# kohjingyu/gill

Measured on AMD Instinct MI355X. Metric: 512x512 images/sec/node, OPT-6.7B+SD1.5 50-step, higher is better.
Workload: dtype bf16

## Files before the change

### gill_amd/csrc/gemm.hip

```cpp
#include "ops.h"
#include <stdlib.h>

#define BM_HOST 128
#define BK 64
#define GEMM_THREADS 256
#define LN_MAX_PLANES 20

#define ZERO_PAGE_STEPS 127
__device__ __attribute__((aligned(256))) uint32_t g_zero_page_storage[(ZERO_PAGE_STEPS + 1) * 32];

const bf16_t* gill_zero_page() {
  static const bf16_t* p = nullptr;
  if (!p) {
    void* d = nullptr;
    if (hipGetSymbolAddress(&d, HIP_SYMBOL(g_zero_page_storage)) == hipSuccess) {
      (void)hipMemset(d, 0, sizeof(g_zero_page_storage));
      p = (const bf16_t*)d;
    }
  }
  return p;
}

struct GemmDev {
  GemmArgs a;
// ... 237 lines not shown

struct GemmTileCtx {
  int bx, by, bz, gdx, gdy;
  unsigned* seam_in = nullptr; unsigned seam_in_target = 0; int seam_in_mtg = 1; int prefetch = 0;
  unsigned* seam_out = nullptr;
};
template <int NWV, int BN, int CONV, int EPI, int STAGES, int KT, int MI, int SEAM = 0>
__device__ __forceinline__ void gemm_tile(const GemmDev& d, const GemmTileCtx cx) {
  constexpr int BM = (NWV / 2) * MI * 16;
  static_assert(MI == 4 || (MI == 2 && NWV == 4 && CONV == 0 && (STAGES == 2 || STAGES == 3) && KT == 64) ||
                    (MI == 2 && NWV == 8 && BN == 160 && STAGES == 3 && KT == 64) || (MI == 2 && NWV == 8 && BN == 64 && STAGES == 6 && CONV == 0 && KT == 64) ||
                    (MI == 2 && NWV == 8 && BN == 128 && STAGES == 2 && CONV == 0 && KT == 64),
                "MI = 2: the 4-wave 64-row plain tile, the 128 x 160 ping-pong tile (8 waves of 32 x 80), or the 128 x 64 streaming tile on 8 waves of 32 x 32");
  constexpr int NT = BN / 32;
  constexpr bool PP = (NWV == 8 && BN == 160 && STAGES == 3 && KT == 64);
  constexpr bool WBLK = (BN == 64 && STAGES == 6 && CONV == 0);
  static_assert(KT == 64 || KT == 32, "stage depth");
  constexpr int LPR = KT / 8;
  constexpr int RPI = 64 / LPR;
  constexpr int KK = KT / 32;
#define SWZ(row) (KT == 64 ? ((row) & 7) : (((row) >> 2) & 3))
  extern __shared__ __attribute__((aligned(16))) unsigned char smem_raw[];
  bf16_t* smem = reinterpret_cast<bf16_t*>(smem_raw);
  constexpr int A_ELEMS = BM * KT;
  constexpr int B_ELEMS = BN * KT;
  constexpr int BUF_ELEMS = A_ELEMS + B_ELEMS;

  const GemmArgs& p = d.a;
  const int tid = threadIdx.x;
  const int lane = tid & 63;
  const int w = __builtin_amdgcn_readfirstlane(tid >> 6);
  int tile;
  {
    const int nwg = cx.gdx, bid = cx.bx;
    const int q = nwg >> 3, r = nwg & 7;
    const int xcd = bid & 7, idx = bid >> 3;
    tile = (xcd < r ? xcd * (q + 1) : r * (q + 1) + (xcd - r) * q) + idx;
  }
  int gn = d.n_major ? tile / d.tiles_m : tile % d.groups_n;
  int tm = d.n_major ? tile % d.tiles_m : tile / d.groups_n;
  if (d.xb_m > 0) {
    const int bid = cx.bx, xcd = bid & 7, idx = bid >> 3;
    const int blocks_m = d.tiles_m / d.xb_m;
    const int bmi = xcd % blocks_m, bni = xcd / blocks_m;
    tm = bmi * d.xb_m + idx % d.xb_m;
    gn = bni * d.xb_n + idx / d.xb_m;
  }
  const int m0 = tm * BM;
  const int tn_first = gn * d.npw;
  const int ntl = (CONV != 0 || EPI == 2 || EPI == 7) ? 1 : ((d.tiles_n - tn_first < d.npw) ? d.tiles_n - tn_first : d.npw);
  int n0 = tn_first * BN;
  const int z = cx.by;
  const int kt_beg = z * d.ksteps_per_split;
  int kt_end = kt_beg + d.ksteps_per_split;
  if (kt_end > d.ksteps) kt_end = d.ksteps;
  const int nsteps = kt_end - kt_beg;
  const int cls = (CONV == 3) ? cx.bz : 0;
  const int ups_py = cls >> 1, ups_px = cls & 1;

  const int srow = lane / LPR;
  const int schunk = (lane % LPR) ^ SWZ(srow);

  constexpr int AI = BM / (RPI * NWV);
  int a_off1[AI], a_off2[AI], a_fl[AI], a_pc[AI];
#pragma unroll
  for (int i = 0; i < AI; ++i) {
    int row = (i * NWV + w) * RPI + srow;
    int m = m0 + row;
    if (m > p.M - 1) m = p.M - 1;
    a_fl[i] = 0; a_pc[i] = 0;
    if constexpr (CONV == 0) {
      a_off1[i] = m * p.lda + schunk * 8;
      a_off2[i] = m * p.lda2 + schunk * 8;
    } else {
      const int ohw = p.OH * p.OW;
      const int b = m / ohw;
      const int r = m - b * ohw;
      const int oy = r / p.OW;
      const int ox = r - oy * p.OW;
      int fl = 0, pc;
      if constexpr (CONV == 3) {
        const int shw = p.IH * p.IW;
        const int sb = m / shw;
        const int sr = m - sb * shw;
        const int sy = sr / p.IW, sx = sr - sy * p.IW;
        pc = m;
        fl |= (sy - 1 >= 0) ? 1 : 0; fl |= (sy + 1 < p.IH) ? 2 : 0;
        fl |= (sx - 1 >= 0) ? 4 : 0; fl |= (sx + 1 < p.IW) ? 8 : 0;
      } else if constexpr (CONV == 2) {
        pc = (b * p.IH + (oy >> 1)) * p.IW + (ox >> 1);
        fl |= (oy - 1 >= 0) ? 1 : 0; fl |= (oy + 1 < p.OH) ? 2 : 0;
        fl |= (ox - 1 >= 0) ? 4 : 0; fl |= (ox + 1 < p.OW) ? 8 : 0;
        fl |= (oy & 1) << 4; fl |= (ox & 1) << 5;
      } else {
        const int cy = oy * p.stride, cx = ox * p.stride;
        pc = (b * p.IH + cy) * p.IW + cx;
        fl |= (cy - 1 >= 0) ? 1 : 0; fl |= (cy + 1 < p.IH) ? 2 : 0;
        fl |= (cx - 1 >= 0) ? 4 : 0; fl |= (cx + 1 < p.IW) ? 8 : 0;
      }
      a_fl[i] = fl;
      a_pc[i] = m;
      a_off1[i] = pc * p.K1 + schunk * 8;
      a_off2[i] = pc * (p.Cin - p.K1) + schunk * 8;
    }
  }
  constexpr int WG = BN / RPI;
  constexpr int WI = (WG + NWV - 1) / NWV;
  static_assert(BN % RPI == 0, "whole row groups");
  const bool w_last_ok = ((WI - 1) * NWV + w) < WG;
  const int lw = AI + (w_last_ok ? WI : WI - 1);
  const bf16_t* w_ptr[WI];
  int n_issue = n0;
  auto tile_col = [&](int R) -> int {
    const int half = R / (BN / 2), q = R - half * (BN / 2);
    const int j = q >> 4, x = q & 15;
    int c;
    if constexpr (EPI == 1) {
      static_assert(EPI != 1 || NT % 4 == 0, "GEGLU: whole value/gate quads per wave");
      const int o = (x >> 2) * 8 + ((j >> 1) & 1) * 4 + (x & 3);
      c = (j >> 2) * 64 + (o >> 4) * 32 + (o & 15) + (j & 1) * 16;
    } else {
      c = ((j | 1) < NT) ? (j >> 1) * 32 + (x >> 2) * 8 + (j & 1) * 4 + (x & 3) : q;
    }
    return half * (BN / 2) + c;
  };
  const bool wblk = WBLK || (CONV == 0 && p.w_blk64 != 0);
  const int w_step = wblk ? 4096 : KT;
  const bf16_t* Wb = p.W + (p.wb_rows ? (size_t)(m0 / p.wb_rows) * (size_t)p.wb_stride : (size_t)0);
  auto w_setup = [&]() {
#pragma unroll
    for (int i = 0; i < WI; ++i) {
      int row = tile_col((i * NWV + w) * RPI + srow);
      int n = n_issue + row;
      if (n > p.N - 1) n = p.N - 1;
      if (wblk) w_ptr[i] = Wb + ((size_t)(n >> 6) * d.ksteps + kt_beg) * 4096 + (n & 63) * 64 + schunk * 8;
      else w_ptr[i] = Wb + ((size_t)cls * p.N + n) * p.K + schunk * 8 + kt_beg * KT;
    }
  };
  w_setup();
  const bf16_t* zero_lane = d.zero + schunk * 8;

  const bf16_t* a_ptr[AI];
  int seg_left = 0;
  auto seg_setup = [&](int k0) {
    if constexpr (CONV == 0) {
      const bool first = (k0 < p.K1);
      const bf16_t* src = first ? p.A : p.A2;
      const int kk = first ? k0 : k0 - p.K1;
#pragma unroll
      for (int i = 0; i < AI; ++i) a_ptr[i] = src + (first ? a_off1[i] : a_off2[i]) + kk;
      seg_left = ((first ? p.K1 : p.K) - k0) / KT;
    } else {
      if (CONV == 1 && k0 >= 9 * p.Cin) {
        const int ke = k0 - 9 * p.Cin;
        const bool fx = (ke < p.KX1);
        const bf16_t* xs = fx ? p.X1 : p.X2;
        const int cx = fx ? p.KX1 : (p.KX - p.KX1);
        const int kc = (fx ? ke : ke - p.KX1) + schunk * 8;
#pragma unroll
        for (int i = 0; i < AI; ++i) a_ptr[i] = xs + (size_t)a_pc[i] * cx + kc;
        seg_left = ((fx ? p.KX1 : p.KX) - ke) / KT;
      } else {
        int tap, c0;
        if (p.k_chunked) {
          const int chunk = k0 / (9 * BK);
          const int r = k0 - chunk * (9 * BK);
          tap = r / BK;
          c0 = chunk * BK + (r - tap * BK);
        } else {
          tap = k0 / p.Cin;
          c0 = k0 - tap * p.Cin;
        }
        const int ty = tap / 3;
        int dy = ty - 1, dx = tap - ty * 3 - 1;
        if constexpr (CONV == 3) { dy = ups_py - 1 + (tap >> 1); dx = ups_px - 1 + (tap & 1); }
        const int need = (dy < 0 ? 1 : (dy > 0 ? 2 : 0)) | (dx < 0 ? 4 : (dx > 0 ? 8 : 0));
        const bool first = (c0 < p.K1);
        const bf16_t* src = first ? p.A : p.A2;
        const int cs = first ? p.K1 : (p.Cin - p.K1);
        const int cc = first ? c0 : c0 - p.K1;
        const int delta = (dy * p.IW + dx) * cs + cc;
#pragma unroll
        for (int i = 0; i < AI; ++i) {
          int off = (first ? a_off1[i] : a_off2[i]);
          if constexpr (CONV == 2) {
            const int ddy = (dy + ((a_fl[i] >> 4) & 1)) >> 1, ddx = (dx + ((a_fl[i] >> 5) & 1)) >> 1;
            off += (ddy * p.IW + ddx) * cs + cc;
          } else {
            off += delta;
          }
          const bool ok = (a_fl[i] & need) == need;
          a_ptr[i] = ok ? src + off : zero_lane;
        }
        seg_left = p.k_chunked ? 1 : ((first ? p.K1 : p.Cin) - c0) / KT;
      }
    }
  };
  int k_issue = kt_beg * KT;
  int steps_in_tile = 0;
  auto issue_prepare = [&]() {
    if (steps_in_tile == nsteps) {
      steps_in_tile = 0;
      k_issue = kt_beg * KT;
      seg_left = 0;
      n_issue += BN;
      w_setup();
    }
    if (seg_left == 0) seg_setup(k_issue);
  };
  auto issue_dma = [&](int buf) {
    bf16_t* As = smem + buf * BUF_ELEMS;
    bf16_t* Bs = As + A_ELEMS;
#pragma unroll
    for (int i = 0; i < AI; ++i) {
      bf16_t* l = As + (i * NWV + w) * RPI * KT;
      __builtin_amdgcn_global_load_lds((const __attribute__((address_space(1))) void*)a_ptr[i],
                                       (__attribute__((address_space(3))) void*)l, 16, 0, 0);
    }
#pragma unroll
    for (int i = 0; i < WI; ++i) {
      if (i == WI - 1 && !w_last_ok) break;
      bf16_t* l = Bs + (i * NWV + w) * RPI * KT;
      __builtin_amdgcn_global_load_lds((const __attribute__((address_space(1))) void*)w_ptr[i],
                                       (__attribute__((address_space(3))) void*)l, 16, 0, WBLK ? 2 : 0);
    }
  };
  auto issue_dma_a = [&](int buf) {
    bf16_t* As = smem + buf * BUF_ELEMS;
#pragma unroll
    for (int i = 0; i < AI; ++i)
      __builtin_amdgcn_global_load_lds((const __attribute__((address_space(1))) void*)a_ptr[i],
                                       (__attribute__((address_space(3))) void*)(As + (i * NWV + w) * RPI * KT), 16, 0, 0);
  };
  auto issue_dma_w = [&](int buf, int koff) {
    bf16_t* Bs = smem + buf * BUF_ELEMS + A_ELEMS;
#pragma unroll
    for (int i = 0; i < WI; ++i) {
      if (i == WI - 1 && !w_last_ok) break;
      __builtin_amdgcn_global_load_lds((const __attribute__((address_space(1))) void*)(w_ptr[i] + koff),
                                       (__attribute__((address_space(3))) void*)(Bs + (i * NWV + w) * RPI * KT), 16, 0, 0);
    }
  };
  auto issue_post = [&]() {
    ++steps_in_tile;
    --seg_left;
#pragma unroll
    for (int i = 0; i < AI; ++i) a_ptr[i] += KT;
#pragma unroll
    for (int i = 0; i < WI; ++i) w_ptr[i] += WBLK ? 4096 : (CONV == 0 ? w_step : KT);
    k_issue += KT;
  };
  auto issue = [&](int buf) {
    issue_prepare();
    issue_dma(buf);
    issue_post();
  };

  f32x4 acc[MI][NT];

  const int wm = w >> 1, wn = w & 1;
  const int frow = lane & 15;
  const int fkc = lane >> 4;

  static_assert(STAGES >= 2 && STAGES <= 6, "ring depth");
  const int total_steps = ntl * nsteps;
  if constexpr (SEAM != 0) {
    static_assert(SEAM == 0 || (PP && !WBLK), "SEAM: the ping-pong tiles");
    if (cx.seam_in) {
      if (cx.prefetch) {
#pragma unroll
        for (int s = 0; s < STAGES - 1; ++s)
          if (s < total_steps) issue_dma_w(s, s * KT);
      }
      if (tid == 0) {
        unsigned* c = cx.seam_in + tm / cx.seam_in_mtg;
        for (unsigned spins = 0; __hip_atomic_load(c, __ATOMIC_RELAXED, __HIP_MEMORY_SCOPE_AGENT) < cx.seam_in_target && spins < COOP_SPIN_LIMIT; ++spins)
          __builtin_amdgcn_s_sleep(2);
        __builtin_amdgcn_fence(__ATOMIC_ACQUIRE, "agent");
      }
      __builtin_amdgcn_s_barrier();
#pragma unroll
      for (int s = 0; s < STAGES - 1; ++s)
        if (s < total_steps) { issue_prepare(); issue_dma_a(s); if (!cx.prefetch) issue_dma_w(s, 0); issue_post(); }
    } else {
#pragma unroll
      for (int s = 0; s < STAGES - 1; ++s)
        if (s < total_steps) issue(s);
    }
  } else {
#pragma unroll
  for (int s = 0; s < STAGES - 1; ++s)
    if (s < total_steps) issue(s);
  }
  float ln_rr[4] = {1.f, 1.f, 1.f, 1.f}, ln_rm[4] = {0.f, 0.f, 0.f, 0.f};
  if constexpr (EPI == 1 || EPI == 3 || EPI == 5) {
    if (p.ln_stats) {
#pragma unroll
      for (int i = 0; i < MI; ++i) {
        const int m = m0 + wm * (MI * 16) + i * 16 + frow;
        if (m < p.M) ln_row_factors(p, m, ln_rr[i], ln_rm[i]);
      }
    }
  }
  int buf = 0, buf_issue = STAGES - 1;
  int flat = 0;
  constexpr bool DEFER = (CONV == 0 && STAGES == 2 && !PP && (EPI == 1 || EPI == 3));
  int deferred_buf = -1;
  for (int t = 0; t < ntl; ++t, n0 += BN) {
#pragma unroll
  for (int i = 0; i < MI; ++i)
#pragma unroll
    for (int j = 0; j < NT; ++j) acc[i][j] = (f32x4){0.f, 0.f, 0.f, 0.f};
  if constexpr (PP) {
    const int grp = w >> 2;
    int issued = total_steps < STAGES - 1 ? total_steps : STAGES - 1;
    bf16x8 af[KK][MI];
    bf16x8 bfr[KK][NT];
    auto landed = [&](int k) {
      if (k >= nsteps) return;
      if constexpr (SEAM != 0) {
        if (cx.seam_in && cx.prefetch && k == 0 && issued == STAGES - 1) { asm volatile("s_waitcnt vmcnt(%0)" ::"n"(AI) : "memory"); return; }
      }
      if (issued - 1 - k <= 0) asm volatile("s_waitcnt vmcnt(0)" ::: "memory");
      else if (w_last_ok) asm volatile("s_waitcnt vmcnt(%0)" ::"n"(AI + WI) : "memory");
      else asm volatile("s_waitcnt vmcnt(%0)" ::"n"(AI + WI - 1) : "memory");
    };
    auto mem = [&](int k) {
      const int sb = k % STAGES;
      const bf16_t* As = smem + sb * BUF_ELEMS;
      const bf16_t* Bs = As + A_ELEMS;
#pragma unroll
      for (int kk = 0; kk < KK; ++kk) {
#pragma unroll
        for (int i = 0; i < MI; ++i) {
          const int row = wm * (MI * 16) + i * 16 + frow;
          af[kk][i] = *reinterpret_cast<const bf16x8*>(As + row * KT + (((kk * 4 + fkc) ^ SWZ(row)) * 8));
        }
#pragma unroll
        for (int j = 0; j < NT; ++j) {
          const int row = wn * (BN / 2) + j * 16 + frow;
          bfr[kk][j] = *reinterpret_cast<const bf16x8*>(Bs + row * KT + (((kk * 4 + fkc) ^ SWZ(row)) * 8));
        }
      }
      if (k + STAGES - 1 < nsteps) { issue_dma((k + STAGES - 1) % STAGES); ++issued; }
    };
    auto mma = [&](int k) {
      issue_post();
#pragma unroll
      for (int kk = 0; kk < KK; ++kk)
#pragma unroll
        for (int i = 0; i < MI; ++i)
#pragma unroll
          for (int j = 0; j < NT; ++j)
            acc[i][j] = __builtin_amdgcn_mfma_f32_16x16x32_bf16(bfr[kk][j], af[kk][i], acc[i][j], 0, 0, 0);
#pragma unroll
      for (int q = 0; q < KK * MI * NT; ++q) {
        __builtin_amdgcn_sched_group_barrier(0x008, 1, 0);
        __builtin_amdgcn_sched_group_barrier(0x006, 1, 0);
      }
      if (k + STAGES < nsteps) issue_prepare();
    };
    if (STAGES - 1 < nsteps) issue_prepare();
    landed(0);
    __builtin_amdgcn_s_barrier();
    if (grp == 0) {
      for (int k = 0; k < nsteps; ++k) {
        mem(k);
        __builtin_amdgcn_sched_barrier(0);
        __builtin_amdgcn_s_barrier();
        mma(k);
        landed(k + 1);
        __builtin_amdgcn_sched_barrier(0);
        __builtin_amdgcn_s_barrier();
      }
      __builtin_amdgcn_s_barrier();
    } else {
      __builtin_amdgcn_s_barrier();
      for (int k = 0; k < nsteps; ++k) {
        mem(k);
        landed(k + 1);
        __builtin_amdgcn_sched_barrier(0);
        __builtin_amdgcn_s_barrier();
        mma(k);
        __builtin_amdgcn_sched_barrier(0);
        __builtin_amdgcn_s_barrier();
      }
    }
  } else
  for (int it = 0; it < nsteps; ++it, ++flat) {
    if constexpr (STAGES == 2) {
      asm volatile("s_waitcnt vmcnt(0)" ::: "memory");
    } else if constexpr (STAGES == 3) {
      if (total_steps - 1 - flat <= 0) asm volatile("s_waitcnt vmcnt(0)" ::: "memory");
      else if (w_last_ok) asm volatile("s_waitcnt vmcnt(%0)" ::"n"(AI + WI) : "memory");
      else asm volatile("s_waitcnt vmcnt(%0)" ::"n"(AI + WI - 1) : "memory");
    } else {
      if (total_steps - 1 - flat < STAGES - 2) asm volatile("s_waitcnt vmcnt(0)" ::: "memory");
      else if (w_last_ok) asm volatile("s_waitcnt vmcnt(%0)" ::"n"((STAGES - 2) * (AI + WI)) : "memory");
      else asm volatile("s_waitcnt vmcnt(%0)" ::"n"((STAGES - 2) * (AI + WI - 1)) : "memory");
    }
    __builtin_amdgcn_s_barrier();
    const bf16_t* As = smem + buf * BUF_ELEMS;
    const bf16_t* Bs = As + A_ELEMS;
    buf = (buf + 1 == STAGES) ? 0 : buf + 1;
    bf16x8 af[KK][MI];
    bf16x8 bfr[KK][NT];
    auto frag_load = [&](int kk) {
#pragma unroll
      for (int i = 0; i < MI; ++i) {
        const int row = wm * (MI * 16) + i * 16 + frow;
        const int slot = (kk * 4 + fkc) ^ SWZ(row);
        af[kk][i] = *reinterpret_cast<const bf16x8*>(As + row * KT + slot * 8);
      }
#pragma unroll
      for (int j = 0; j < NT; ++j) {
        const int row = wn * (BN / 2) + j * 16 + frow;
        const int slot = (kk * 4 + fkc) ^ SWZ(row);
        bfr[kk][j] = *reinterpret_cast<const bf16x8*>(Bs + row * KT + slot * 8);
      }
    };
    frag_load(0);
    if (flat + STAGES - 1 < total_steps) {
      if (DEFER && it == nsteps - 1) deferred_buf = buf_issue;
      else issue(buf_issue);
    }
    buf_issue = (buf_issue + 1 == STAGES) ? 0 : buf_issue + 1;
#pragma unroll
    for (int kk = 0; kk < KK; ++kk) {
      if (kk + 1 < KK) {
        __builtin_amdgcn_sched_barrier(0);
        frag_load(kk + 1);
        __builtin_amdgcn_sched_barrier(0);
      }
#pragma unroll
      for (int i = 0; i < MI; ++i)
#pragma unroll
        for (int j = 0; j < NT; ++j)
          acc[i][j] = __builtin_amdgcn_mfma_f32_16x16x32_bf16(bfr[kk][j], af[kk][i], acc[i][j], 0, 0, 0);
    }
  }

  const int mrow = m0 + wm * (MI * 16) + frow;
  const int nbase = n0 + wn * (BN / 2);
  constexpr int NG = (NT + 1) / 2;
  auto out_row = [&](int m) -> int {
    if constexpr (CONV == 3) {
      const int shw = p.IH * p.IW;
      const int sb = m / shw;
      const int sr = m - sb * shw;
      const int sy = sr / p.IW, sx = sr - sy * p.IW;
      return (sb * p.OH + 2 * sy + ups_py) * p.OW + 2 * sx + ups_px;
    } else {
      return m;
    }
  };
  if constexpr (EPI == 2 || EPI == 7) {
    float* ws = p.ws + (size_t)z * (CONV == 3 ? 4 : 1) * p.M * p.N;
#pragma unroll
    for (int i = 0; i < MI; ++i) {
      if (mrow + i * 16 >= p.M) continue;
      const int m = out_row(mrow + i * 16);
#pragma unroll
      for (int g = 0; g < NG; ++g) {
        const bool pair = (2 * g + 1 < NT);
        const int j1 = pair ? 2 * g + 1 : 2 * g;
        const int n = nbase + (pair ? g * 32 + fkc * 8 : (2 * g) * 16 + fkc * 4);
        if (n >= p.N) continue;
        float* dst = ws + (size_t)m * p.N + n;
        if constexpr (EPI == 7) {
          st_wt_f32x4(dst, acc[i][2 * g]);
          if (pair && n + 4 < p.N) st_wt_f32x4(dst + 4, acc[i][j1]);
        } else {
          *reinterpret_cast<float4*>(dst) = make_float4(acc[i][2 * g][0], acc[i][2 * g][1], acc[i][2 * g][2], acc[i][2 * g][3]);
          if (pair && n + 4 < p.N)
            *reinterpret_cast<float4*>(dst + 4) = make_float4(acc[i][j1][0], acc[i][j1][1], acc[i][j1][2], acc[i][j1][3]);
        }
      }
    }
    if constexpr (EPI == 7) {
      static_assert(EPI != 7 || (PP && BN % 40 == 0), "COOP split-K finish: the ping-pong tiles");
      asm volatile("s_waitcnt vmcnt(0)" ::: "memory");
      __syncthreads();
      const int rpb = p.rows_per_batch;
      const int mtg = rpb > BM ? rpb / BM : 1, spg = rpb < BM ? BM / rpb : 1;
      const int G = mtg * cx.gdy;
      const int tg = tm / mtg;
      unsigned char* cs = smem_raw + 16384;
      float2 (*part)[10] = reinterpret_cast<float2 (*)[10]>(cs);
      float2* quad = reinterpret_cast<float2*>(cs + 2048);
      float2* mr = reinterpret_cast<float2*>(cs + 2304);
      unsigned* okf = reinterpret_cast<unsigned*>(cs + 2560);
      if (tid == 0) {
        const bool ok = coop_arrive_wait(p.coop_ctr + (size_t)tg * d.tiles_n + n0 / BN, (unsigned)G);
        __builtin_amdgcn_fence(__ATOMIC_ACQUIRE, "agent");
        *okf = ok ? 1u : 0u;
      }
      __syncthreads();
      const bool poison = *okf == 0u;
      constexpr int UPT = BN / 40;
      const int widx = z * mtg + (tm - tg * mtg);
      for (int u = widx; u < spg * UPT; u += G) {
        const int b = tg * spg + u / UPT, col0 = n0 + (u % UPT) * 40;
        if (rpb == 256) splitk_finish_unit<16, 40>(p, b, col0, tid, part, quad, mr, poison);
        else splitk_finish_unit<4, 40>(p, b, col0, tid, part, quad, mr, poison);
        __syncthreads();
      }
      if constexpr (SEAM != 0) {
        if (cx.seam_out) {
          asm volatile("s_waitcnt vmcnt(0)" ::: "memory");
          __syncthreads();
          if (tid == 0) {
            __builtin_amdgcn_fence(__ATOMIC_RELEASE, "agent");
            asm volatile("s_waitcnt vmcnt(0)" ::: "memory");
            __hip_atomic_fetch_add(cx.seam_out + tg, 1u, __ATOMIC_RELAXED, __HIP_MEMORY_SCOPE_AGENT);
          }
        }
      }
    }
  } else if constexpr (EPI == 1) {
    const float* rr = ln_rr; const float* rm = ln_rm;
#pragma unroll
    for (int qd = 0; qd < NT / 4; ++qd) {
      const int ol = fkc * 8;
      const int pv = nbase + qd * 64 + (ol >> 4) * 32 + (ol & 15);
      if (nbase + qd * 64 >= p.N) continue;
      const int no = (nbase + qd * 64) / 2 + ol;
      float4 bv[2], bg[2], sv[2], sg[2];
#pragma unroll
      for (int h = 0; h < 2; ++h) {
        bv[h] = p.bias ? *reinterpret_cast<const float4*>(p.bias + pv + 4 * h) : make_float4(0, 0, 0, 0);
        bg[h] = p.bias ? *reinterpret_cast<const float4*>(p.bias + pv + 16 + 4 * h) : make_float4(0, 0, 0, 0);
        sv[h] = p.ln_stats ? *reinterpret_cast<const float4*>(p.ln_colsum + pv + 4 * h) : make_float4(0, 0, 0, 0);
        sg[h] = p.ln_stats ? *reinterpret_cast<const float4*>(p.ln_colsum + pv + 16 + 4 * h) : make_float4(0, 0, 0, 0);
      }
      __builtin_amdgcn_s_waitcnt(0x0F70);
      if (DEFER && qd == NT / 4 - 1 && deferred_buf >= 0) { issue(deferred_buf); deferred_buf = -1; }
#pragma unroll
      for (int i = 0; i < MI; ++i) {
        const int m = mrow + i * 16;
        float o[8];
#pragma unroll
        for (int h = 0; h < 2; ++h) {
          const f32x4 av = acc[i][qd * 4 + 2 * h], ag = acc[i][qd * 4 + 2 * h + 1];
          o[4 * h + 0] = (av[0] * rr[i] - rm[i] * sv[h].x + bv[h].x) * gelu_erf(ag[0] * rr[i] - rm[i] * sg[h].x + bg[h].x);
          o[4 * h + 1] = (av[1] * rr[i] - rm[i] * sv[h].y + bv[h].y) * gelu_erf(ag[1] * rr[i] - rm[i] * sg[h].y + bg[h].y);
          o[4 * h + 2] = (av[2] * rr[i] - rm[i] * sv[h].z + bv[h].z) * gelu_erf(ag[2] * rr[i] - rm[i] * sg[h].z + bg[h].z);
          o[4 * h + 3] = (av[3] * rr[i] - rm[i] * sv[h].w + bv[h].w) * gelu_erf(ag[3] * rr[i] - rm[i] * sg[h].w + bg[h].w);
        }
        uint4 ov; ov.x = pack_bf2(o[0], o[1]); ov.y = pack_bf2(o[2], o[3]); ov.z = pack_bf2(o[4], o[5]); ov.w = pack_bf2(o[6], o[7]);
        if (m < p.M) *reinterpret_cast<uint4*>((bf16_t*)p.C + (size_t)m * p.ldc + no) = ov;
      }
    }
  } else if constexpr (EPI == 5) {
    static_assert(EPI != 5 || BN == 160, "softmax epilogue: one 80-column head per wave half");
    const size_t vb = p.wb_rows ? (size_t)(m0 / p.wb_rows) * (size_t)p.vb_stride : (size_t)0;
    const float* bias = p.bias + vb;
    const float* csum = p.ln_colsum + vb;
    float4 bzs[NG][2], css[NG][2];
#pragma unroll
    for (int g = 0; g < NG; ++g) {
      const bool pair = (2 * g + 1 < NT);
      const int n = nbase + (pair ? g * 32 + fkc * 8 : (2 * g) * 16 + fkc * 4);
      bzs[g][0] = *reinterpret_cast<const float4*>(bias + n);
      css[g][0] = *reinterpret_cast<const float4*>(csum + n);
      bzs[g][1] = pair ? *reinterpret_cast<const float4*>(bias + n + 4) : make_float4(0, 0, 0, 0);
      css[g][1] = pair ? *reinterpret_cast<const float4*>(csum + n + 4) : make_float4(0, 0, 0, 0);
    }
    __builtin_amdgcn_s_waitcnt(0x0F70);
#pragma unroll
    for (int i = 0; i < MI; ++i) {
      const int m = mrow + i * 16;
      const float rr = ln_rr[i], rm = ln_rm[i];
      float v[NG][8];
      float mx = -INFINITY;
#pragma unroll
      for (int g = 0; g < NG; ++g) {
        const bool pair = (2 * g + 1 < NT);
        const f32x4 a0 = acc[i][2 * g], a1 = acc[i][pair ? 2 * g + 1 : 2 * g];
        v[g][0] = a0[0] * rr - rm * css[g][0].x + bzs[g][0].x; v[g][1] = a0[1] * rr - rm * css[g][0].y + bzs[g][0].y;
        v[g][2] = a0[2] * rr - rm * css[g][0].z + bzs[g][0].z; v[g][3] = a0[3] * rr - rm * css[g][0].w + bzs[g][0].w;
        v[g][4] = pair ? a1[0] * rr - rm * css[g][1].x + bzs[g][1].x : -INFINITY; v[g][5] = pair ? a1[1] * rr - rm * css[g][1].y + bzs[g][1].y : -INFINITY;
        v[g][6] = pair ? a1[2] * rr - rm * css[g][1].z + bzs[g][1].z : -INFINITY; v[g][7] = pair ? a1[3] * rr - rm * css[g][1].w + bzs[g][1].w : -INFINITY;
#pragma unroll
        for (int e = 0; e < 8; ++e) mx = fmaxf(mx, v[g][e]);
      }
      mx = fmaxf(mx, __shfl_xor(mx, 16, 64));
      mx = fmaxf(mx, __shfl_xor(mx, 32, 64));
      float sum = 0.f;
#pragma unroll
      for (int g = 0; g < NG; ++g)
#pragma unroll
        for (int e = 0; e < 8; ++e) { v[g][e] = __builtin_amdgcn_exp2f(v[g][e] - mx); sum += v[g][e]; }
      sum += __shfl_xor(sum, 16, 64);
      sum += __shfl_xor(sum, 32, 64);
      const float inv = 1.f / sum;
      if (m < p.M) {
        bf16_t* crow = (bf16_t*)p.C + (size_t)m * p.ldc;
#pragma unroll
        for (int g = 0; g < NG; ++g) {
          const bool pair = (2 * g + 1 < NT);
          const int n = nbase + (pair ? g * 32 + fkc * 8 : (2 * g) * 16 + fkc * 4);
          uint4 o; o.x = pack_bf2(v[g][0] * inv, v[g][1] * inv); o.y = pack_bf2(v[g][2] * inv, v[g][3] * inv);
          o.z = pack_bf2(v[g][4] * inv, v[g][5] * inv); o.w = pack_bf2(v[g][6] * inv, v[g][7] * inv);
          if (pair) *reinterpret_cast<uint4*>(crow + n) = o;
          else *reinterpret_cast<uint2*>(crow + n) = make_uint2(o.x, o.y);
        }
      }
    }
  } else if constexpr (EPI == 3) {
    int rq[MI], rk[MI], rv[MI]; bool mok[MI];
    float rr[MI], rm[MI];
#pragma unroll
    for (int i = 0; i < MI; ++i) {
      const int m = mrow + i * 16;
      mok[i] = m < p.M;
      rr[i] = p.ln_stats ? ln_rr[i] : p.alpha; rm[i] = ln_rm[i];
      const int b = m / p.ntok, t = m - b * p.ntok;
      rq[i] = (b * p.heads * p.ntok_pad_q + t) * p.dp;
      rk[i] = (b * p.heads * p.ntok_pad_kv + t + p.kv_tok_offset) * p.dp;
      rv[i] = b * p.heads * p.dpv * p.ntok_pad_kv + t + p.kv_tok_offset;
    }
    const int hd = p.heads * p.dp;
    float4 bzs[NG][2], css[NG][2];
#pragma unroll
    for (int g = 0; g < NG; ++g) {
      const bool pair = (2 * g + 1 < NT);
      const int n = nbase + (pair ? g * 32 + fkc * 8 : (2 * g) * 16 + fkc * 4);
      const bool hi = pair && (n + 4 < p.N);
#pragma unroll
      for (int e = 0; e < 2; ++e) {
        const bool ok = (n < p.N) && ((e == 0) || hi);
        bzs[g][e] = (p.bias && ok) ? *reinterpret_cast<const float4*>(p.bias + n + 4 * e) : make_float4(0, 0, 0, 0);
        css[g][e] = (p.ln_stats && ok) ? *reinterpret_cast<const float4*>(p.ln_colsum + n + 4 * e) : make_float4(0, 0, 0, 0);
      }
    }
    __builtin_amdgcn_s_waitcnt(0x0F70);
    if (DEFER && deferred_buf >= 0) { issue(deferred_buf); deferred_buf = -1; }
#pragma unroll
    for (int g = 0; g < NG; ++g) {
      const bool pair = (2 * g + 1 < NT);
      const int j1 = pair ? 2 * g + 1 : 2 * g;
      const int n = nbase + (pair ? g * 32 + fkc * 8 : (2 * g) * 16 + fkc * 4);
      if (n >= p.N) continue;
      const bool hi = pair && (n + 4 < p.N);
      const int segl = n / hd;
      const int within = n - segl * hd;
      const int h = within / p.dp, dd = within - h * p.dp;
      const int seg = p.seg_base + segl;
      const float4* bz = bzs[g]; const float4* cs = css[g];
#pragma unroll
      for (int i = 0; i < MI; ++i) {
        if (!mok[i]) continue;
        float v[8];
        const f32x4 a0 = acc[i][2 * g], a1 = acc[i][j1];
        v[0] = a0[0] * rr[i] - rm[i] * cs[0].x + bz[0].x; v[1] = a0[1] * rr[i] - rm[i] * cs[0].y + bz[0].y;
        v[2] = a0[2] * rr[i] - rm[i] * cs[0].z + bz[0].z; v[3] = a0[3] * rr[i] - rm[i] * cs[0].w + bz[0].w;
        v[4] = a1[0] * rr[i] - rm[i] * cs[1].x + bz[1].x; v[5] = a1[1] * rr[i] - rm[i] * cs[1].y + bz[1].y;
        v[6] = a1[2] * rr[i] - rm[i] * cs[1].z + bz[1].z; v[7] = a1[3] * rr[i] - rm[i] * cs[1].w + bz[1].w;
        if (seg == 0) {
#pragma unroll
          for (int e = 0; e < 8; ++e) v[e] *= p.qscale;
        }
        if (seg <= 1) {
          bf16_t* dst = (seg == 0) ? p.Cq + (size_t)rq[i] + (size_t)h * p.ntok_pad_q * p.dp + dd
                                   : p.Ck + (size_t)rk[i] + (size_t)h * p.ntok_pad_kv * p.dp + dd;
          if (hi) {
            uint4 o; o.x = pack_bf2(v[0], v[1]); o.y = pack_bf2(v[2], v[3]); o.z = pack_bf2(v[4], v[5]); o.w = pack_bf2(v[6], v[7]);
            *reinterpret_cast<uint4*>(dst) = o;
          } else {
            uint2 o; o.x = pack_bf2(v[0], v[1]); o.y = pack_bf2(v[2], v[3]);
            *reinterpret_cast<uint2*>(dst) = o;
          }
        } else {
          bf16_t* base = p.Cvt + (size_t)rv[i] + (size_t)(h * p.dpv + dd) * p.ntok_pad_kv;
          const int ne = hi ? 8 : 4;
#pragma unroll
          for (int e = 0; e < 8; ++e)
            if (e < ne) base[(size_t)e * p.ntok_pad_kv] = f2bf(v[e]);
          if (dd + ne == p.dp && p.dpv > p.dp) base[(size_t)ne * p.ntok_pad_kv] = (bf16_t)0x3F80;
        }
      }
    }
  } else {
    int crow[MI], rrow[MI]; bool mok[MI];
#pragma unroll
    for (int i = 0; i < MI; ++i) {
      const int m = mrow + i * 16;
      mok[i] = m < p.M;
      const int mc = mok[i] ? m : p.M - 1;
      crow[i] = out_row(mc) * p.ldc;
      rrow[i] = mc * p.ldr;
    }
    float2* red = reinterpret_cast<float2*>(smem);
    float2* red_lane = red + wm * BN + wn * (BN / 2);
    if (p.gn_stats) __syncthreads();
    float rws[4] = {0.f, 0.f, 0.f, 0.f}, rwq[4] = {0.f, 0.f, 0.f, 0.f};
    constexpr bool F32_PATHS = (CONV == 0 && EPI != 4);
    constexpr bool ALL_UPFRONT = !F32_PATHS;
    constexpr int NSLOT = ALL_UPFRONT ? NG : 1;
    const int wrow0 = m0 + wm * (MI * 16);
    const int wrow1 = (wrow0 + MI * 16 - 1 < p.M) ? wrow0 + MI * 16 - 1 : p.M - 1;
    const bool rv_pre = p.rowvec && wrow0 < p.M && (wrow0 / p.rows_per_batch == wrow1 / p.rows_per_batch);
    const bool rv_slow = p.rowvec && !rv_pre;
    const bool rf_slow = F32_PATHS && p.resid && p.resid_f32;
    const bool rb_pre = p.resid && !rf_slow;
    const float* colvec = rv_pre ? p.rowvec + (wrow0 / p.rows_per_batch) * p.rowvec_bstride : p.bias;
    const float* colvec2 = rv_pre ? p.bias : nullptr;
    float4 cv[NSLOT][2];
    uint2 rb[NSLOT][MI][2];
    auto load_group = [&](int g, int sl) {
      const bool pair = (2 * g + 1 < NT);
      const int n = nbase + (pair ? g * 32 + fkc * 8 : (2 * g) * 16 + fkc * 4);
      const bool hi = pair && (n + 4 < p.N);
      const int nl = (n < p.N) ? n : 0;
      const int nh = hi ? n + 4 : nl;
      cv[sl][0] = cv[sl][1] = make_float4(0, 0, 0, 0);
      if (colvec) {
        cv[sl][0] = *reinterpret_cast<const float4*>(colvec + nl);
        cv[sl][1] = *reinterpret_cast<const float4*>(colvec + nh);
      }
      if (colvec2) {
        const float4 t0 = *reinterpret_cast<const float4*>(colvec2 + nl);
        const float4 t1 = *reinterpret_cast<const float4*>(colvec2 + nh);
        cv[sl][0].x += t0.x; cv[sl][0].y += t0.y; cv[sl][0].z += t0.z; cv[sl][0].w += t0.w;
        cv[sl][1].x += t1.x; cv[sl][1].y += t1.y; cv[sl][1].z += t1.z; cv[sl][1].w += t1.w;
      }
    };
    auto load_group_resid = [&](int g, int sl) {
      const bool pair = (2 * g + 1 < NT);
      const int n = nbase + (pair ? g * 32 + fkc * 8 : (2 * g) * 16 + fkc * 4);
      const bool hi = pair && (n + 4 < p.N);
      const int nl = (n < p.N) ? n : 0;
      const int nh = hi ? n + 4 : nl;
#pragma unroll
      for (int i = 0; i < MI; ++i) {
        rb[sl][i][0] = *reinterpret_cast<const uint2*>((const bf16_t*)p.resid + rrow[i] + nl);
        rb[sl][i][1] = *reinterpret_cast<const uint2*>((const bf16_t*)p.resid + rrow[i] + nh);
      }
    };
    if constexpr (ALL_UPFRONT) {
#pragma unroll
      for (int g = 0; g < NG; ++g) load_group(g, g);
      if (rb_pre) {
#pragma unroll
        for (int g = 0; g < NG; ++g) load_group_resid(g, g);
      }
      __builtin_amdgcn_s_waitcnt(0x0F70);
    }
#pragma unroll
    for (int g = 0; g < NG; ++g) {
      const int sl = ALL_UPFRONT ? g : 0;
      const int rs = sl;
      if constexpr (!ALL_UPFRONT) {
        load_group(g, 0);
        if (rb_pre) load_group_resid(g, 0);
        __builtin_amdgcn_s_waitcnt(0x0F70);
      }
      const bool pair = (2 * g + 1 < NT);
      const int j1 = pair ? 2 * g + 1 : 2 * g;
      const int cl = pair ? g * 32 + fkc * 8 : (2 * g) * 16 + fkc * 4;
      const int n = nbase + cl;
      const bool nok = n < p.N;
      const bool hi = pair && (n + 4 < p.N);
      float gs[8] = {0.f, 0.f, 0.f, 0.f, 0.f, 0.f, 0.f, 0.f}, gq[8] = {0.f, 0.f, 0.f, 0.f, 0.f, 0.f, 0.f, 0.f};
#pragma unroll
      for (int i = 0; i < MI; ++i) {
        const f32x4 a0 = acc[i][2 * g], a1 = acc[i][j1];
        float v[8] = {a0[0] * p.alpha + cv[sl][0].x, a0[1] * p.alpha + cv[sl][0].y, a0[2] * p.alpha + cv[sl][0].z, a0[3] * p.alpha + cv[sl][0].w,
                      a1[0] * p.alpha + cv[sl][1].x, a1[1] * p.alpha + cv[sl][1].y, a1[2] * p.alpha + cv[sl][1].z, a1[3] * p.alpha + cv[sl][1].w};
        if (rv_slow) {
          const int vr = (min(mrow + i * 16, p.M - 1) / p.rows_per_batch) * p.rowvec_bstride;
          const int nl = nok ? n : 0, nh = hi ? n + 4 : nl;
          const float4 b0 = *reinterpret_cast<const float4*>(p.rowvec + vr + nl);
          const float4 b1 = *reinterpret_cast<const float4*>(p.rowvec + vr + nh);
          v[0] += b0.x; v[1] += b0.y; v[2] += b0.z; v[3] += b0.w;
          v[4] += b1.x; v[5] += b1.y; v[6] += b1.z; v[7] += b1.w;
        }
        if (rb_pre) {
          v[0] += bf2f((bf16_t)(rb[rs][i][0].x & 0xffff)); v[1] += bf2f((bf16_t)(rb[rs][i][0].x >> 16));
          v[2] += bf2f((bf16_t)(rb[rs][i][0].y & 0xffff)); v[3] += bf2f((bf16_t)(rb[rs][i][0].y >> 16));
          v[4] += bf2f((bf16_t)(rb[rs][i][1].x & 0xffff)); v[5] += bf2f((bf16_t)(rb[rs][i][1].x >> 16));
          v[6] += bf2f((bf16_t)(rb[rs][i][1].y & 0xffff)); v[7] += bf2f((bf16_t)(rb[rs][i][1].y >> 16));
        }
        if (F32_PATHS && rf_slow) {
          const int nl = nok ? n : 0, nh = hi ? n + 4 : nl;
          const float4 r0 = *reinterpret_cast<const float4*>((const float*)p.resid + rrow[i] + nl);
          const float4 r1 = *reinterpret_cast<const float4*>((const float*)p.resid + rrow[i] + nh);
          v[0] += r0.x; v[1] += r0.y; v[2] += r0.z; v[3] += r0.w;
          v[4] += r1.x; v[5] += r1.y; v[6] += r1.z; v[7] += r1.w;
        }
        if (F32_PATHS && p.act != ACT_NONE) {
#pragma unroll
          for (int e = 0; e < 8; ++e) v[e] = apply_act(v[e], p.act);
        }
        const bool st = mok[i] && nok;
        if (F32_PATHS && p.out_mode == OUT_F32) {
          if (st) *reinterpret_cast<float4*>((float*)p.C + crow[i] + n) = make_float4(v[0], v[1], v[2], v[3]);
          if (st && hi) *reinterpret_cast<float4*>((float*)p.C + crow[i] + n + 4) = make_float4(v[4], v[5], v[6], v[7]);
        } else {
          uint4 o; o.x = pack_bf2(v[0], v[1]); o.y = pack_bf2(v[2], v[3]); o.z = pack_bf2(v[4], v[5]); o.w = pack_bf2(v[6], v[7]);
          const bool stc = st && EPI != 6;
          if (stc && hi) *reinterpret_cast<uint4*>((bf16_t*)p.C + crow[i] + n) = o;
          else if (stc) *reinterpret_cast<uint2*>((bf16_t*)p.C + crow[i] + n) = make_uint2(o.x, o.y);
          if constexpr (EPI == 6) {
            acc[i][2 * g] = (f32x4){v[0], v[1], v[2], v[3]};
            if (pair) acc[i][j1] = (f32x4){v[4], v[5], v[6], v[7]};
          }
          if (CONV == 0 && p.row_stats) {
            const float r0 = __uint_as_float(o.x << 16), r1 = __uint_as_float(o.x & 0xffff0000u);
            const float r2 = __uint_as_float(o.y << 16), r3 = __uint_as_float(o.y & 0xffff0000u);
            const float r4 = __uint_as_float(o.z << 16), r5 = __uint_as_float(o.z & 0xffff0000u);
            const float r6 = __uint_as_float(o.w << 16), r7 = __uint_as_float(o.w & 0xffff0000u);
            const float slo = (r0 + r1) + (r2 + r3), qlo = (r0 * r0 + r1 * r1) + (r2 * r2 + r3 * r3);
            const float shi = (r4 + r5) + (r6 + r7), qhi = (r4 * r4 + r5 * r5) + (r6 * r6 + r7 * r7);
            rws[i] += nok ? slo : 0.f;
            rwq[i] += nok ? qlo : 0.f;
            rws[i] += hi ? shi : 0.f;
            rwq[i] += hi ? qhi : 0.f;
          }
        }
#pragma unroll
        for (int e = 0; e < 8; ++e) {
          const float ve = mok[i] ? v[e] : 0.f;
          gs[e] += ve; gq[e] += ve * ve;
        }
      }
      if (p.gn_stats) {
#pragma unroll
        for (int e = 0; e < 8; ++e) {
          if (e >= 4 && !pair) break;
          const float a = row16_sum(gs[e]), q = row16_sum(gq[e]);
          if (frow == 0) red_lane[cl + e] = make_float2(a, q);
        }
      }
    }
    if (CONV == 0 && p.row_stats) {
      float* plane = p.row_stats + (size_t)((n0 / BN) * 2 + wn) * p.M * 2;
#pragma unroll
      for (int i = 0; i < MI; ++i) {
        rws[i] += __shfl_xor(rws[i], 16, 64); rwq[i] += __shfl_xor(rwq[i], 16, 64);
        rws[i] += __shfl_xor(rws[i], 32, 64); rwq[i] += __shfl_xor(rwq[i], 32, 64);
        if (fkc == 0 && mok[i]) *reinterpret_cast<float2*>(plane + (size_t)(mrow + i * 16) * 2) = make_float2(rws[i], rwq[i]);
      }
    }
    if (p.gn_stats) {
      __syncthreads();
      constexpr int HALVES = BM / 64;
      const int bins_tile = BN / p.gn_cg;
      if (tid < 2 * HALVES * bins_tile) {
        const int which = tid & 1, half = (tid >> 1) % HALVES, lb = (tid >> 1) / HALVES;
        const int mfirst = m0 + half * 64;
        const int bin = n0 / p.gn_cg + lb;
        if (mfirst < p.M && bin < p.gn_groups) {
          constexpr int GPS = 64 / (MI * 16);
          float a = 0.f;
#pragma unroll
          for (int g = 0; g < GPS; ++g) {
            const float* src = reinterpret_cast<const float*>(red + (half * GPS + g) * BN + lb * p.gn_cg) + which;
            for (int c = 0; c < p.gn_cg; ++c) a += src[2 * c];
          }
          const int b = mfirst / p.rows_per_batch;
          const int slab = (mfirst - b * p.rows_per_batch) / GN_SLAB_ROWS + (CONV == 3 ? cls * (p.rows_per_batch / GN_SLAB_ROWS) : 0);
          const int nslab = (CONV == 3 ? 4 : 1) * (p.rows_per_batch / GN_SLAB_ROWS);
          float* dst = p.gn_stats + (((size_t)b * nslab + slab) * p.gn_groups + bin) * 2 + which;
          if constexpr (EPI == 6) st_wt_f32(dst, a);
          else *dst = a;
        }
      }
    }
    if constexpr (EPI == 6) {
      static_assert(EPI != 6 || (PP && CONV == 1), "COOP GroupNorm finish: the ping-pong convolution tiles");
      asm volatile("s_waitcnt vmcnt(0)" ::: "memory");
      __syncthreads();
      float* cs = reinterpret_cast<float*>(smem_raw + 16384);
      float* c_seg = cs; float* c_tot = cs + 256; float* c_sc = cs + 320; float* c_sh = cs + 320 + BN; unsigned* okf = reinterpret_cast<unsigned*>(cs + 320 + 2 * BN);
      const int bsmp = m0 / p.rows_per_batch;
      unsigned* gctr = p.coop_ctr + (size_t)bsmp * d.tiles_n + n0 / BN;
      if (tid == 0) coop_arrive(gctr);
      const bool colt = tid < BN && n0 + tid < p.N;
      const float gam_c = colt ? p.fn_gamma[n0 + tid] : 0.f, bet_c = colt ? p.fn_beta[n0 + tid] : 0.f;
      if (p.C) {
#pragma unroll
        for (int g = 0; g < NG; ++g) {
          const bool pair = (2 * g + 1 < NT);
          const int j1 = pair ? 2 * g + 1 : 2 * g;
          const int n = nbase + (pair ? g * 32 + fkc * 8 : (2 * g) * 16 + fkc * 4);
          const bool nok = n < p.N;
          const bool hi = pair && (n + 4 < p.N);
#pragma unroll
          for (int i = 0; i < MI; ++i) {
            const f32x4 a0 = acc[i][2 * g], a1 = acc[i][j1];
            uint4 o; o.x = pack_bf2(a0[0], a0[1]); o.y = pack_bf2(a0[2], a0[3]); o.z = pack_bf2(a1[0], a1[1]); o.w = pack_bf2(a1[2], a1[3]);
            if (mok[i] && nok && hi) *reinterpret_cast<uint4*>((bf16_t*)p.C + crow[i] + n) = o;
            else if (mok[i] && nok) *reinterpret_cast<uint2*>((bf16_t*)p.C + crow[i] + n) = make_uint2(o.x, o.y);
          }
        }
      }
      if (tid == 0) {
        const bool ok = coop_wait(gctr, (unsigned)(p.rows_per_batch / BM));
        *okf = ok ? 1u : 0u;
      }
      __syncthreads();
      const bool ok = *okf != 0u;
      const int bins_tile = BN / p.gn_cg;
      const int ns = p.rows_per_batch / GN_SLAB_ROWS;
      if (tid < bins_tile * 8) {
        const int seg = tid & 3, which = (tid >> 2) & 1, lb = tid >> 3;
        const float* src = p.gn_stats + (((size_t)bsmp * ns + seg * 16) * p.gn_groups + n0 / p.gn_cg + lb) * 2 + which;
        const size_t step = (size_t)p.gn_groups * 2;
        float pv[16];
#pragma unroll
        for (int i = 0; i < 16; ++i) pv[i] = (seg * 16 + i < ns) ? ld_wt_f32(src + (size_t)i * step) : 0.f;
        c_seg[(lb * 2 + which) * 4 + seg] = (((pv[0] + pv[1]) + (pv[2] + pv[3])) + ((pv[4] + pv[5]) + (pv[6] + pv[7]))) +
                                            (((pv[8] + pv[9]) + (pv[10] + pv[11])) + ((pv[12] + pv[13]) + (pv[14] + pv[15])));
      }
      __syncthreads();
      if (tid < bins_tile * 2) { const float* g4 = c_seg + tid * 4; c_tot[tid] = (g4[0] + g4[1]) + (g4[2] + g4[3]); }
      __syncthreads();
      if (tid < BN && n0 + tid < p.N) {
        const int gl = tid / p.fn_cg, r1 = p.fn_cg / p.gn_cg;
        float a = 0.f, q = 0.f;
        for (int bin = gl * r1; bin < (gl + 1) * r1; ++bin) { a += c_tot[bin * 2]; q += c_tot[bin * 2 + 1]; }
        const float inv_n = 1.f / ((float)p.fn_cg * (float)p.rows_per_batch);
        const float sm = a * inv_n;
        const float sq = q * inv_n;
        const float var = fmaxf(sq - sm * sm, 0.f);
        const float rstd = rsqrtf(var + p.fn_eps);
        float sc = rstd * gam_c;
        if (!ok) sc = __builtin_nanf("");
        const float sh = bet_c - sm * sc;
        c_sc[tid] = sc; c_sh[tid] = sh;
        if (p.fn_ss && m0 == bsmp * p.rows_per_batch) {
          p.fn_ss[((size_t)bsmp * 2 + 0) * p.N + n0 + tid] = sc;
          p.fn_ss[((size_t)bsmp * 2 + 1) * p.N + n0 + tid] = sh;
        }
      }
      __syncthreads();
      if (p.fn_Y) {
#pragma unroll
        for (int g = 0; g < NG; ++g) {
          const bool pair = (2 * g + 1 < NT);
          const int j1 = pair ? 2 * g + 1 : 2 * g;
          const int cl = pair ? g * 32 + fkc * 8 : (2 * g) * 16 + fkc * 4;
          const int n = nbase + cl;
          const bool nok = n < p.N;
          const bool hi = pair && (n + 4 < p.N);
          const float* scp = c_sc + wn * (BN / 2) + cl; const float* shp = c_sh + wn * (BN / 2) + cl;
          const float4 s0 = *reinterpret_cast<const float4*>(scp), h0 = *reinterpret_cast<const float4*>(shp);
          const float4 s1 = pair ? *reinterpret_cast<const float4*>(scp + 4) : s0, h1 = pair ? *reinterpret_cast<const float4*>(shp + 4) : h0;
#pragma unroll
          for (int i = 0; i < MI; ++i) {
            const f32x4 a0 = acc[i][2 * g], a1 = acc[i][j1];
            float o[8];
            o[0] = fmaf(bf2f(f2bf(a0[0])), s0.x, h0.x); o[1] = fmaf(bf2f(f2bf(a0[1])), s0.y, h0.y);
            o[2] = fmaf(bf2f(f2bf(a0[2])), s0.z, h0.z); o[3] = fmaf(bf2f(f2bf(a0[3])), s0.w, h0.w);
            o[4] = fmaf(bf2f(f2bf(a1[0])), s1.x, h1.x); o[5] = fmaf(bf2f(f2bf(a1[1])), s1.y, h1.y);
            o[6] = fmaf(bf2f(f2bf(a1[2])), s1.z, h1.z); o[7] = fmaf(bf2f(f2bf(a1[3])), s1.w, h1.w);
            if (p.fn_silu) {
#pragma unroll
              for (int e = 0; e < 8; ++e) o[e] = silu_f(o[e]);
            }
            uint4 ov; ov.x = pack_bf2(o[0], o[1]); ov.y = pack_bf2(o[2], o[3]); ov.z = pack_bf2(o[4], o[5]); ov.w = pack_bf2(o[6], o[7]);
            bf16_t* yrow = p.fn_Y + (size_t)(mrow + i * 16) * p.N + n;
            if (mok[i] && nok && hi) *reinterpret_cast<uint4*>(yrow) = ov;
            else if (mok[i] && nok) *reinterpret_cast<uint2*>(yrow) = make_uint2(ov.x, ov.y);
          }
        }
      }
    }
  }
  }
#undef SWZ
}
template <int NWV, int BN, int CONV, int EPI, int STAGES, int KT, int MI>
__global__ __launch_bounds__(NWV * 64, NWV == 8 ? ((BN == 128 && STAGES == 2) ? 2 : 1) : (MI == 2 ? 3 : 2)) void gemm_kernel(const GemmDev d) {
  kernarg_warm<sizeof(GemmDev)>();
  GemmTileCtx cx;
  cx.bx = blockIdx.x; cx.by = blockIdx.y; cx.bz = blockIdx.z; cx.gdx = gridDim.x; cx.gdy = gridDim.y;
  gemm_tile<NWV, BN, CONV, EPI, STAGES, KT, MI, 0>(d, cx);
}

template <int W, int R>
__global__ __launch_bounds__(4 * W) void gemm_splitk_reduce_kernel(const GemmArgs p) {
  kernarg_warm<sizeof(GemmArgs)>();
  constexpr int QW = W / 4;
  constexpr int ROWS = 16 * R;
  __shared__ float2 rowp[ROWS][QW];
  __shared__ float2 colp[16][W];
  const int tx = threadIdx.x % QW, ty = threadIdx.x / QW;
  const int n = blockIdx.x * W + tx * 4;
  const int mbase = blockIdx.y * ROWS;
  float gs[4] = {0.f, 0.f, 0.f, 0.f}, gq[4] = {0.f, 0.f, 0.f, 0.f};
  float rsum[R], rsq[R];
#pragma unroll
  for (int r = 0; r < R; ++r) { rsum[r] = 0.f; rsq[r] = 0.f; }
  auto row_of = [&](int r) -> int { return mbase + ty + 16 * r; };
  if (n < p.N) {
    float4 s[R];
    const float* src[R];
#pragma unroll
    for (int r = 0; r < R; ++r) {
      int m = mbase + ty + 16 * r;
      if (m > p.M - 1) m = p.M - 1;
      s[r] = make_float4(0, 0, 0, 0);
      src[r] = p.ws + (size_t)m * p.N + n;
    }
    const size_t zstride = (size_t)p.M * p.N;
    constexpr int U = 16 / R;
    int z = 0;
    for (; z + U <= p.splitk; z += U) {
      float4 v[R][U];
#pragma unroll
      for (int r = 0; r < R; ++r)
#pragma unroll
        for (int u = 0; u < U; ++u) v[r][u] = *reinterpret_cast<const float4*>(src[r] + (size_t)(z + u) * zstride);
#pragma unroll
      for (int r = 0; r < R; ++r)
#pragma unroll
        for (int u = 0; u < U; ++u) { s[r].x += v[r][u].x; s[r].y += v[r][u].y; s[r].z += v[r][u].z; s[r].w += v[r][u].w; }
    }
    for (; z < p.splitk; ++z) {
      float4 v[R];
#pragma unroll
      for (int r = 0; r < R; ++r) v[r] = *reinterpret_cast<const float4*>(src[r] + (size_t)z * zstride);
#pragma unroll
      for (int r = 0; r < R; ++r) { s[r].x += v[r].x; s[r].y += v[r].y; s[r].z += v[r].z; s[r].w += v[r].w; }
    }
    const float4 cs = p.ln_stats ? *reinterpret_cast<const float4*>(p.ln_colsum + n) : make_float4(0, 0, 0, 0);
#pragma unroll
    for (int r = 0; r < R; ++r) {
      const int m = row_of(r);
      if (m >= p.M) continue;
      if (p.ln_stats) {
        float rr, rm;
        ln_row_factors(p, m, rr, rm);
        s[r].x = s[r].x * rr - rm * cs.x; s[r].y = s[r].y * rr - rm * cs.y;
        s[r].z = s[r].z * rr - rm * cs.z; s[r].w = s[r].w * rr - rm * cs.w;
      }
      float fin[4];
      store4(p, m, n, s[r].x, s[r].y, s[r].z, s[r].w, fin);
#pragma unroll
      for (int e = 0; e < 4; ++e) { gs[e] += fin[e]; gq[e] += fin[e] * fin[e]; }
#pragma unroll
      for (int e = 0; e < 4; ++e) { const float q = bf2f(f2bf(fin[e])); rsum[r] += q; rsq[r] += q * q; }
    }
  }
  if (p.row_stats) {
#pragma unroll
    for (int r = 0; r < R; ++r) rowp[ty + 16 * r][tx] = make_float2(rsum[r], rsq[r]);
    __syncthreads();
// ... 509 lines not shown
```

Before: 8.642.

## Prefetch epilogue bias and residual tiles into LDS during final K-steps

In the pipelined GEMM path, the epilogue's column-vector (bias/rowvec) and bf16 residual loads are issued as async global-to-LDS DMA into free ring-buffer slots during the last main-loop iterations. The epilogue then reads them from shared memory instead of issuing global loads after the MMA loop, hiding that load latency behind compute. Wait counts are adjusted so the outstanding prefetches don't stall the final K steps, and the gn_stats barrier is moved after the LDS reads. This adds complexity and depends on alignment and ring-slot reuse being correct.

```diff
diff --git a/gill_amd/csrc/gemm.hip b/gill_amd/csrc/gemm.hip
--- a/gill_amd/csrc/gemm.hip
+++ b/gill_amd/csrc/gemm.hip
@@ -563,6 +563,52 @@
       }
     }
   }
+  auto epi_colvecs = [&](const float*& colvec, const float*& colvec2) -> bool {
+    const int wrow0 = m0 + wm * (MI * 16);
+    const int wrow1 = (wrow0 + MI * 16 - 1 < p.M) ? wrow0 + MI * 16 - 1 : p.M - 1;
+    const bool rv_pre = p.rowvec && wrow0 < p.M && (wrow0 / p.rows_per_batch == wrow1 / p.rows_per_batch);
+    colvec = rv_pre ? p.rowvec + (wrow0 / p.rows_per_batch) * p.rowvec_bstride : p.bias;
+    colvec2 = rv_pre ? p.bias : nullptr;
+    return rv_pre;
+  };
+  constexpr bool PF = PP && SEAM == 0 && (EPI == 0 || EPI == 4 || EPI == 6) && !(CONV == 0 && EPI != 4) && !(CONV == 0 && MI == 4);
+  constexpr int PF_RI = MI * 16 * (BN / 2) * 2 / 1024;
+  constexpr int PF_R0 = (PF_RI + 1) / 2, PF_R1 = PF_RI / 2;
+  constexpr int PF_CVU = BN / 2 / 4;
+  constexpr int PF_CV_OFF = NWV * PF_R0 * 1024;
+  static_assert(!PF || (PF_RI * 1024 == MI * 16 * (BN / 2) * 2 && 2 * PF_CVU <= 64 && 64 % (MI * 16) == 0), "PF: whole pieces");
+  static_assert(!PF || (PF_CV_OFF + NWV * 1024 <= BUF_ELEMS * 2 && NWV * PF_R1 * 1024 <= BUF_ELEMS * 2), "PF: the staged operands fit a ring slot");
+  const bool pf = PF && nsteps >= 2 && (p.N & 7) == 0;
+  const bool pf_rb = pf && p.resid && (p.ldr & 7) == 0 && ((uintptr_t)p.resid & 15) == 0;
+  auto pf_issue = [&](int part) {
+    int ln;
+    asm volatile("v_mov_b32 %0, %1" : "=v"(ln) : "v"(lane));
+    unsigned char* base = smem_raw + ((nsteps + part) % STAGES) * (BUF_ELEMS * (int)sizeof(bf16_t));
+    const int nb = n0 + wn * (BN / 2);
+    if (pf_rb) {
+      int m = m0 + wm * (MI * 16) + ln % (MI * 16);
+      if (m > p.M - 1) m = p.M - 1;
+      const bf16_t* rrp = (const bf16_t*)p.resid + m * p.ldr;
+#pragma unroll
+      for (int j = 0; j < PF_RI; ++j) {
+        if ((j < PF_R0) != (part == 0)) continue;
+        const int c = nb + ((j * 64 + ln) / (MI * 16)) * 8;
+        unsigned char* l = base + (w * (part == 0 ? PF_R0 : PF_R1) + (part == 0 ? j : j - PF_R0)) * 1024;
+        __builtin_amdgcn_global_load_lds((const __attribute__((address_space(1))) void*)(rrp + (c < p.N ? c : 0)),
+                                         (__attribute__((address_space(3))) void*)l, 16, 0, 0);
+      }
+    }
+    if (part == 0) {
+      const float* colvec; const float* colvec2;
+      epi_colvecs(colvec, colvec2);
+      const int q = ln < PF_CVU ? ln : ln - PF_CVU;
+      const float* src = ln < PF_CVU ? colvec : (ln < 2 * PF_CVU ? colvec2 : nullptr);
+      const int c = nb + 4 * q;
+      const void* a = src ? (const void*)(src + (c < p.N ? c : 0)) : (const void*)d.zero;
+      __builtin_amdgcn_global_load_lds((const __attribute__((address_space(1))) void*)a,
+                                       (__attribute__((address_space(3))) void*)(base + PF_CV_OFF + w * 1024), 16, 0, 0);
+    }
+  };
   int buf = 0, buf_issue = STAGES - 1;
   int flat = 0;
   constexpr bool DEFER = (CONV == 0 && STAGES == 2 && !PP && (EPI == 1 || EPI == 3));
@@ -582,7 +628,13 @@
       if constexpr (SEAM != 0) {
         if (cx.seam_in && cx.prefetch && k == 0 && issued == STAGES - 1) { asm volatile("s_waitcnt vmcnt(%0)" ::"n"(AI) : "memory"); return; }
       }
-      if (issued - 1 - k <= 0) asm volatile("s_waitcnt vmcnt(0)" ::: "memory");
+      if (issued - 1 - k <= 0) {
+        if constexpr (PF) {
+          if (pf_rb) { asm volatile("s_waitcnt vmcnt(%0)" ::"n"(PF_R0 + 1) : "memory"); return; }
+          if (pf) { asm volatile("s_waitcnt vmcnt(1)" ::: "memory"); return; }
+        }
+        asm volatile("s_waitcnt vmcnt(0)" ::: "memory");
+      }
       else if (w_last_ok) asm volatile("s_waitcnt vmcnt(%0)" ::"n"(AI + WI) : "memory");
       else asm volatile("s_waitcnt vmcnt(%0)" ::"n"(AI + WI - 1) : "memory");
     };
@@ -604,6 +656,10 @@
         }
       }
       if (k + STAGES - 1 < nsteps) { issue_dma((k + STAGES - 1) % STAGES); ++issued; }
+      if constexpr (PF) {
+        if (pf && k + STAGES - 1 == nsteps) pf_issue(0);
+        if (pf && k + STAGES - 1 == nsteps + 1) pf_issue(1);
+      }
     };
     auto mma = [&](int k) {
       issue_post();
@@ -954,19 +1010,16 @@
     }
     float2* red = reinterpret_cast<float2*>(smem);
     float2* red_lane = red + wm * BN + wn * (BN / 2);
-    if (p.gn_stats) __syncthreads();
+    if (p.gn_stats && !pf) __syncthreads();
     float rws[4] = {0.f, 0.f, 0.f, 0.f}, rwq[4] = {0.f, 0.f, 0.f, 0.f};
     constexpr bool F32_PATHS = (CONV == 0 && EPI != 4);
     constexpr bool ALL_UPFRONT = !F32_PATHS;
     constexpr int NSLOT = ALL_UPFRONT ? NG : 1;
-    const int wrow0 = m0 + wm * (MI * 16);
-    const int wrow1 = (wrow0 + MI * 16 - 1 < p.M) ? wrow0 + MI * 16 - 1 : p.M - 1;
-    const bool rv_pre = p.rowvec && wrow0 < p.M && (wrow0 / p.rows_per_batch == wrow1 / p.rows_per_batch);
+    const float* colvec; const float* colvec2;
+    const bool rv_pre = epi_colvecs(colvec, colvec2);
     const bool rv_slow = p.rowvec && !rv_pre;
     const bool rf_slow = F32_PATHS && p.resid && p.resid_f32;
     const bool rb_pre = p.resid && !rf_slow;
-    const float* colvec = rv_pre ? p.rowvec + (wrow0 / p.rows_per_batch) * p.rowvec_bstride : p.bias;
-    const float* colvec2 = rv_pre ? p.bias : nullptr;
     float4 cv[NSLOT][2];
     uint2 rb[NSLOT][MI][2];
     auto load_group = [&](int g, int sl) {
@@ -999,14 +1052,57 @@
         rb[sl][i][1] = *reinterpret_cast<const uint2*>((const bf16_t*)p.resid + rrow[i] + nh);
       }
     };
+    const unsigned char* pf_x = smem_raw + (nsteps % STAGES) * (BUF_ELEMS * (int)sizeof(bf16_t));
+    const unsigned char* pf_y = smem_raw + ((nsteps + 1) % STAGES) * (BUF_ELEMS * (int)sizeof(bf16_t));
+    auto pf_group = [&](int g) {
+      const bool pair = (2 * g + 1 < NT);
+      const int cl = pair ? g * 32 + fkc * 8 : (2 * g) * 16 + fkc * 4;
+      const int n = nbase + cl;
+      const bool nok = n < p.N;
+      const bool hi = pair && (n + 4 < p.N);
+      const float* cvs = reinterpret_cast<const float*>(pf_x + PF_CV_OFF + w * 1024);
+      const int u0 = cl >> 2, u1 = hi ? u0 + 1 : u0;
+      cv[g][0] = cv[g][1] = make_float4(0, 0, 0, 0);
+      if (colvec) {
+        cv[g][0] = *reinterpret_cast<const float4*>(cvs + u0 * 4);
+        cv[g][1] = *reinterpret_cast<const float4*>(cvs + u1 * 4);
+      }
+      if (colvec2) {
+        const float4 t0 = *reinterpret_cast<const float4*>(cvs + (PF_CVU + u0) * 4);
+        const float4 t1 = *reinterpret_cast<const float4*>(cvs + (PF_CVU + u1) * 4);
+        cv[g][0].x += t0.x; cv[g][0].y += t0.y; cv[g][0].z += t0.z; cv[g][0].w += t0.w;
+        cv[g][1].x += t1.x; cv[g][1].y += t1.y; cv[g][1].z += t1.z; cv[g][1].w += t1.w;
+      }
+      if (pf_rb) {
+#pragma unroll
+        for (int i = 0; i < MI; ++i) {
+          const int u = (cl >> 3) * (MI * 16) + i * 16 + frow;
+          const unsigned char* a = (u < PF_R0 * 64) ? pf_x + (w * PF_R0 * 64 + u) * 16 : pf_y + (w * PF_R1 * 64 + u - PF_R0 * 64) * 16;
+          if (pair) {
+            const uint4 r = *reinterpret_cast<const uint4*>(a);
+            rb[g][i][0] = make_uint2(r.x, r.y);
+            rb[g][i][1] = hi ? make_uint2(r.z, r.w) : make_uint2(r.x, r.y);
+          } else {
+            rb[g][i][0] = rb[g][i][1] = *reinterpret_cast<const uint2*>(a + (nok ? (cl & 7) * 2 : 0));
+          }
+        }
+      }
+    };
     if constexpr (ALL_UPFRONT) {
-#pragma unroll
-      for (int g = 0; g < NG; ++g) load_group(g, g);
-      if (rb_pre) {
+      if (pf) {
+        asm volatile("s_waitcnt vmcnt(0)" ::: "memory");
+#pragma unroll
+        for (int g = 0; g < NG; ++g) pf_group(g);
+      } else {
+#pragma unroll
+        for (int g = 0; g < NG; ++g) load_group(g, g);
+      }
+      if (rb_pre && !pf_rb) {
 #pragma unroll
         for (int g = 0; g < NG; ++g) load_group_resid(g, g);
       }
       __builtin_amdgcn_s_waitcnt(0x0F70);
+      if (p.gn_stats && pf) __syncthreads();
     }
 #pragma unroll
     for (int g = 0; g < NG; ++g) {
```

Measured after the change: 8.477, median of 2. -1.9%, worse.
